# mabdullahsoyturk/Torch-Sputnik

Measured on AMD Instinct MI355X. Metric: SpMM effective GFLOP/s (2*nnz*N/t), M=N=K=4096 fp32, density 0.1, higher is better.
Workload: dtype f32

## Files before the change

torch_sputnik_amd/csrc/gen_spmm_flat.py:

```python
#!/usr/bin/env python3
import argparse

_ap = argparse.ArgumentParser()
_ap.add_argument("--mode", default="entry", choices=["entry", "group"])
_ap.add_argument("--layout", default="straight", choices=["straight", "diagonal"])
_ap.add_argument("out", nargs="?")
ARGS = _ap.parse_args()
GROUP = ARGS.mode == "group"

BK = 32
BK_SHIFT = 5
ROW_BYTES = 2048
ROW_SHIFT = 11
WIN_BYTES = 144
NSTRIP = 4
NPIECES = 4
ROWSTEP = 8

V_LANE, V_STAGE, V_PLAN, V_ROWS = "v0", "v1", "v2", "v3"
CUR_OFF, CUR_VAL = 4, 5
NXT_OFF, NXT_VAL, NXT_ROWS = 6, 7, 8
NN_OFF, NN_VAL, NN_ROWS = 10, 11, 12
PAIR = [16, 18, 20, 22]
VALT = [16, 18]
V_ADDR = 20
STRIP = [32, 40, 48, 56]
ACC = 64

S_STREAM, S_VALUES, S_CINFO, S_DENSE = "s[36:37]", "s[38:39]", "s[40:41]", "s[42:43]"
S_PITCH, S_KMAX, S_NCHUNKS, S_ROW0, S_LDS0, S_DEBUG = "s44", "s45", "s46", "s47", "s48", "s49"
S_REM, S_C, S_CIOFF, S_MINE, S_SB, S_NSW = "s50", "s51", "s56", "s57", "s76", "s77"
S_CI = ["s52", "s53", "s54", "s55"]
S_RET, S_BND = "s[58:59]", "s[60:61]"
S_ROWS = [62, 63, 64, 65]
S_IDX = [66, 67, 68, 69]
S_COLS = "s78"
S_T = ["s70", "s71", "s72", "s73", "s74", "s75"]

out = []


def emit(line):
    out.append(line)


def label(name):
    return f".L_{name}_%="


def strip_reads(ring, addr):
    s = STRIP[ring]
    emit(f"ds_read_b128 v[{s}:{s + 3}], v{addr}")
    emit(f"ds_read_b128 v[{s + 4}:{s + 7}], v{addr} offset:1024")


def fmas(src_pair, op_sel, ring):
    s = STRIP[ring]
    for q in range(4):
        emit(f"v_pk_fma_f32 v[{ACC + 2 * q}:{ACC + 2 * q + 1}], v[{src_pair}:{src_pair + 1}], "
             f"v[{s + 2 * q}:{s + 2 * q + 1}], v[{ACC + 2 * q}:{ACC + 2 * q + 1}] {op_sel}")


def entry_fma_stage(ring, lgkm):
    emit(f"s_waitcnt lgkmcnt({lgkm})")
    emit(f"s_set_gpr_idx_on s{S_IDX[ring]}, 0xc")
    fmas(PAIR[ring], "op_sel:[1,0,0] op_sel_hi:[1,1,1]", ring)
    emit("s_set_gpr_idx_off")


def entry_slot(slot):
    ring = slot % NSTRIP
    p = PAIR[ring]
    emit(f"{label(f'E_{slot}')}:")
    emit(f"s_sub_u32 {S_REM}, {S_REM}, 1")
    emit(f"s_cbranch_scc1 {label(f'bnd_{slot}')}")
    emit(f"v_mov_b64_dpp v[{p}:{p + 1}], v[{CUR_OFF}:{CUR_VAL}] row_newbcast:{slot} row_mask:0xf bank_mask:0xf")
    emit(f"s_bfe_u32 s{S_IDX[ring]}, s{S_ROWS[slot // 4]}, {hex(8 * (slot % 4) | (7 << 16))}")
    emit(f"v_add_u32 v{p}, v{p}, {V_LANE}")
    strip_reads(ring, p)
    entry_fma_stage((ring + 1) % NSTRIP, 2 * (NSTRIP - 1))


def group_entry_body(ring, slot):
    t = VALT[slot % 2]
    emit(f"v_mov_b32_dpp v{t}, v{CUR_VAL} row_newbcast:{slot} row_mask:0xf bank_mask:0xf")
    emit(f"s_bfe_u32 s{S_IDX[0]}, s{S_ROWS[slot // 4]}, {hex(8 * (slot % 4) | (7 << 16))}")
    emit(f"s_set_gpr_idx_on s{S_IDX[0]}, 0xc")
    fmas(t, "op_sel:[0,0,0] op_sel_hi:[0,1,1]", ring)
    emit("s_set_gpr_idx_off")


def group_start(ring, slot):
    emit(f"{label(f'N_{ring}_{slot}')}:")
    emit(f"s_sub_u32 {S_REM}, {S_REM}, 1")
    emit(f"s_cbranch_scc1 {label(f'bnd_{slot}')}")
    emit(f"v_mov_b32_dpp v{V_ADDR}, v{CUR_OFF} row_newbcast:{slot} row_mask:0xf bank_mask:0xf")
    emit(f"v_add_u32 v{V_ADDR}, v{V_ADDR}, {V_LANE}")
    strip_reads(ring, V_ADDR)
    emit(f"s_waitcnt lgkmcnt({2 * (NSTRIP - 1)})")


def first_groups():
    for i in range(NSTRIP - 1):
        emit(f"s_bfe_u32 {S_T[0]}, {S_COLS}, {hex(8 * i | (8 << 16))}")
        emit(f"s_lshl_b32 {S_T[0]}, {S_T[0]}, {ROW_SHIFT}")
        emit(f"v_add_u32 v{V_ADDR}, {S_T[0]}, {V_LANE}")
        strip_reads(i, V_ADDR)


def stage_chunk(chunk_sgpr):
    t_row, t_lds, t_r, t_lo, t_hi = S_T[1], S_T[2], S_T[3], S_T[4], S_T[5]
    emit(f"s_lshl_b32 {t_row}, {chunk_sgpr}, {BK_SHIFT}")
    emit(f"s_add_u32 {t_row}, {t_row}, {S_ROW0}")
    emit(f"s_and_b32 {t_lds}, {chunk_sgpr}, 1")
    emit(f"s_lshl_b32 {t_lds}, {t_lds}, 16")
    emit(f"s_add_u32 {t_lds}, {t_lds}, {S_LDS0}")
    for i in range(NPIECES):
        emit(f"s_add_u32 {t_r}, {t_row}, {ROWSTEP * i}")
        emit(f"s_min_u32 {t_r}, {t_r}, {S_KMAX}")
        emit(f"s_mul_hi_u32 {t_hi}, {t_r}, {S_PITCH}")
        emit(f"s_mul_i32 {t_lo}, {t_r}, {S_PITCH}")
        emit(f"s_add_u32 {t_lo}, {t_lo}, s42")
        emit(f"s_addc_u32 {t_hi}, {t_hi}, s43")
        emit(f"s_add_u32 m0, {t_lds}, {hex(ROWSTEP * i * ROW_BYTES)}")
        emit("s_nop 0")
        emit(f"global_load_lds_dwordx4 {V_STAGE}, s[{t_lo[1:]}:{t_hi[1:]}]")


def plan_load(off, rows):
    emit(f"global_load_dwordx2 v[{off}:{off + 1}], {V_PLAN}, {S_STREAM}")
    emit(f"global_load_dword v{rows}, {V_ROWS}, {S_STREAM}")
    emit(f"v_add_u32 {V_PLAN}, {hex(WIN_BYTES)}, {V_PLAN}")
    emit(f"v_add_u32 {V_ROWS}, {hex(WIN_BYTES)}, {V_ROWS}")


def gather(val):
    emit(f"global_load_dword v{val}, v{val}, {S_VALUES}")


def switch_window(tag):
    emit(f"s_cmp_lg_u32 {S_SB}, 0")
    emit(f"s_cbranch_scc1 {label('swc_' + tag)}")
    emit("s_waitcnt vmcnt(0)")
    emit(f"s_branch {label('swd_' + tag)}")
    emit(f"{label('swc_' + tag)}:")
    emit(f"s_waitcnt vmcnt({NPIECES})")
    emit(f"{label('swd_' + tag)}:")
    emit(f"s_mov_b32 {S_SB}, 0")
    emit(f"s_add_u32 {S_NSW}, {S_NSW}, 1")
    for i in range(4):
        emit(f"v_readlane_b32 s{S_ROWS[i]}, v{NXT_ROWS}, {i}")
    emit(f"v_bfe_u32 v{CUR_OFF}, v{NXT_OFF}, {8 if GROUP else 0}, 8")
    emit(f"v_mov_b32 v{CUR_VAL}, v{NXT_VAL}")
    emit(f"v_lshlrev_b32 v{CUR_OFF}, {ROW_SHIFT}, v{CUR_OFF}")
    emit(f"v_mov_b64 v[{NXT_OFF}:{NXT_VAL}], v[{NN_OFF}:{NN_VAL}]")
    emit(f"v_mov_b32 v{NXT_ROWS}, v{NN_ROWS}")
    emit(f"s_bitcmp1_b32 {S_DEBUG}, 3")
    emit(f"s_cbranch_scc1 {label('swskip_' + tag)}")
    gather(NXT_VAL)
    plan_load(NN_OFF, NN_ROWS)
    emit(f"{label('swskip_' + tag)}:")
    emit("s_nop 1")


def take_chunk_info():
    emit(f"s_mov_b32 {S_REM}, {S_CI[0] if GROUP else S_CI[3]}")
    if GROUP:
        emit(f"s_mov_b32 {S_COLS}, {S_CI[1]}")


def generate():
    emit("; ---- prologue ----")
    for r in list(range(ACC, ACC + 64)) + list(range(STRIP[0], STRIP[0] + 32)) + list(range(16, 24)):
        emit(f"v_mov_b32 v{r}, 0")
    for r in S_IDX:
        emit(f"s_mov_b32 s{r}, 0")
    emit(f"s_getpc_b64 {S_BND}")
    emit(f"{label('pc')}:")
    emit(f"s_add_u32 s60, s60, {label('boundary')}-{label('pc')}")
    emit("s_addc_u32 s61, s61, 0")
    plan_load(NXT_OFF, NXT_ROWS)
    plan_load(NN_OFF, NN_ROWS)
    emit("s_waitcnt vmcnt(2)")
    gather(NXT_VAL)
    emit(f"s_mov_b32 {S_T[0]}, 0")
    stage_chunk(S_T[0])
    emit(f"s_load_dwordx4 s[52:55], {S_CINFO}, 0x0")
    emit("s_waitcnt vmcnt(0) lgkmcnt(0)")
    emit("s_barrier")
    take_chunk_info()
    emit(f"s_load_dwordx4 s[52:55], {S_CINFO}, 0x10")
    emit(f"s_mov_b32 {S_CIOFF}, 32")
    emit(f"s_mov_b32 {S_C}, 0")
    emit(f"s_mov_b32 {S_NSW}, 0")
    emit(f"s_mov_b32 {S_SB}, 0")
    emit(f"s_mov_b32 {S_MINE}, 0")
    if GROUP:
        first_groups()
    emit(f"s_cmp_lt_u32 {S_NCHUNKS}, 2")
    emit(f"s_cbranch_scc1 {label('pro_nostage')}")
    emit(f"s_mov_b32 {S_T[0]}, 1")
    stage_chunk(S_T[0])
    emit(f"s_mov_b32 {S_SB}, 1")
    emit(f"s_mov_b32 {S_MINE}, 1")
    emit(f"{label('pro_nostage')}:")
    switch_window("pro")

    emit("; ---- main loop ----")
    if not GROUP:
        for slot in range(16):
            entry_slot(slot)
        switch_window("w")
        emit(f"s_branch {label('E_0')}")
    elif ARGS.layout == "straight":
        emit(f"s_branch {label(f'E_{NSTRIP - 1}_0')}")
        for ring in range(NSTRIP):
            for slot in range(16):
                emit(f"{label(f'E_{ring}_{slot}')}:")
                emit(f"s_bitcmp1_b32 s{S_ROWS[slot // 4]}, {8 * (slot % 4) + 7}")
                emit(f"s_cbranch_scc1 {label(f'N_{ring}_{slot}')}")
                emit(f"{label(f'B_{ring}_{slot}')}:")
                group_entry_body(ring, slot)
            switch_window(f"r{ring}")
            emit(f"s_branch {label(f'E_{ring}_0')}")
        emit("; ---- first entry of a column group ----")
        for ring in range(NSTRIP):
            for slot in range(16):
                group_start(ring, slot)
                emit(f"s_branch {label(f'B_{(ring + 1) % NSTRIP}_{slot}')}")
    else:
        emit(f"s_branch {label(f'E_{NSTRIP - 1}_0')}")
        for diag in range(NSTRIP):
            for slot in range(16):
                ring = (diag + slot) % NSTRIP
                emit(f"{label(f'E_{ring}_{slot}')}:")
                emit(f"s_bitcmp1_b32 s{S_ROWS[slot // 4]}, {8 * (slot % 4) + 7}")
                emit(f"s_cbranch_scc0 {label(f'B_{ring}_{slot}')}")
                group_start(ring, slot)
                emit(f"{label(f'B_{(ring + 1) % NSTRIP}_{slot}')}:")
                group_entry_body((ring + 1) % NSTRIP, slot)
            ring = (diag + 16) % NSTRIP
            switch_window(f"r{diag}")
            emit(f"s_branch {label(f'E_{ring}_0')}")

    emit("; ---- boundary stubs ----")
    for slot in range(16):
        emit(f"{label(f'bnd_{slot}')}:")
        emit(f"s_swappc_b64 {S_RET}, {S_BND}")
        if GROUP:
            emit(f"s_cbranch_scc1 {label('end')}")
            emit(f"s_branch {label(f'N_{NSTRIP - 1}_{slot}')}")
        else:
            emit(f"s_cbranch_scc1 {label(f'drain_{slot % NSTRIP}')}")
            emit(f"s_branch {label(f'E_{slot}')}")

    emit("; ---- boundary subroutine ----")
    emit(f"{label('boundary')}:")
    emit(f"s_bitcmp1_b32 {S_DEBUG}, 2")
    emit(f"s_cbranch_scc1 {label('bnodrain')}")
    emit("s_waitcnt lgkmcnt(0)")
    emit(f"{label('bnodrain')}:")
    emit(f"s_cmp_eq_u32 {S_MINE}, 0")
    emit(f"s_cbranch_scc1 {label('bvd')}")
    emit(f"s_bitcmp1_b32 {S_DEBUG}, 5")
    emit(f"s_cbranch_scc1 {label('bvd')}")
    for n in range(3):
        emit(f"s_cmp_eq_u32 {S_NSW}, {n}")
        emit(f"s_cbranch_scc1 {label(f'bv{n}')}")
    emit("s_waitcnt vmcnt(9)")
    emit(f"s_branch {label('bvd')}")
    for n in range(3):
        emit(f"{label(f'bv{n}')}:")
        emit(f"s_waitcnt vmcnt({3 * n})")
        if n < 2:
            emit(f"s_branch {label('bvd')}")
    emit(f"{label('bvd')}:")
    emit(f"s_bitcmp1_b32 {S_DEBUG}, 1")
    emit(f"s_cbranch_scc1 {label('bnobar')}")
    emit("s_barrier")
    emit(f"{label('bnobar')}:")
    emit(f"s_add_u32 {S_C}, {S_C}, 1")
    emit(f"s_cmp_eq_u32 {S_C}, {S_NCHUNKS}")
    emit(f"s_cbranch_scc1 {label('bret')}")
    take_chunk_info()
    emit(f"s_load_dwordx4 s[52:55], {S_CINFO}, {S_CIOFF}")
    emit(f"s_add_u32 {S_CIOFF}, {S_CIOFF}, 16")
    if GROUP:
        first_groups()
    emit(f"s_mov_b32 {S_NSW}, 0")
    emit(f"s_mov_b32 {S_MINE}, 0")
    emit(f"s_add_u32 {S_T[0]}, {S_C}, 1")
    emit(f"s_cmp_ge_u32 {S_T[0]}, {S_NCHUNKS}")
    emit(f"s_cbranch_scc1 {label('bnostage')}")
    emit(f"s_bitcmp1_b32 {S_DEBUG}, 0")
    emit(f"s_cbranch_scc1 {label('bnostage')}")
    stage_chunk(S_T[0])
    emit(f"s_add_u32 {S_SB}, {S_SB}, 1")
    emit(f"s_mov_b32 {S_MINE}, 1")
    emit(f"{label('bnostage')}:")
    emit(f"s_cmp_eq_u32 {S_C}, {S_NCHUNKS}")
    emit(f"{label('bret')}:")
    emit(f"s_setpc_b64 {S_RET}")

    if not GROUP:
        emit("; ---- drain: the three entries still in the pipeline ----")
        for ring in range(NSTRIP):
            emit(f"{label(f'drain_{ring}')}:")
            for j in range(1, NSTRIP):
                entry_fma_stage((ring + j) % NSTRIP, 2 * (NSTRIP - 1 - j))
            if ring < NSTRIP - 1:
                emit(f"s_branch {label('end')}")
    emit(f"{label('end')}:")
    emit("s_waitcnt vmcnt(0) lgkmcnt(0)")


def main():
    generate()
    text = "// GENERATED by gen_spmm_flat.py -- do not edit.\n" + "".join(
        f'"{line}\\n"\n' for line in out)
    if ARGS.out:
        with open(ARGS.out, "w") as f:
            f.write(text)
    else:
        print(text, end="")


if __name__ == "__main__":
    main()
```

torch_sputnik_amd/csrc/spmm_flat.hip:

```cpp
#include <algorithm>

#include "options.h"
#include "spmm_tiled_common.h"

namespace sputnik_hip {

namespace {

using namespace tiled;

constexpr int kBN = 512;
constexpr int kBK = 32;
constexpr int kWaves = 16;
constexpr int kRPW = 8;
constexpr int kBM = kWaves * kRPW;
constexpr int kAhead = 3;
constexpr int kDealPer = 256;
constexpr int kWindow = 16;
constexpr int kWindowBytes = 144;
constexpr int kTailWindows = 4;
constexpr int kMaxColumns = 65536;
constexpr unsigned kNewGroup = 0x80;


struct ChunkInfo {
  int groups;
  unsigned first_rows;
  unsigned unused;
  int entries;
};

__host__ __device__ inline size_t fill_tables_bytes(int nchunks) {
  return (sizeof(int) * (static_cast<size_t>(nchunks) * (kBK / 4 + 4) + 2 * kRPW + 2) + 15) / 16 * 16;
}
__device__ __forceinline__ int wave_sum(int v) {
#pragma unroll
  for (int o = 32; o > 0; o >>= 1) v += __shfl_xor(v, o);
  return v;
}
__device__ __forceinline__ int wave_inclusive_scan(int v, int lane) {
#pragma unroll
  for (int o = 1; o < 64; o <<= 1) {
    const int t = __shfl_up(v, o);
    if (lane >= o) v += t;
  }
  return v;
}

__global__ __launch_bounds__(kRPW * 64) void spmm_flat_fill_kernel(
    int m, int k, int slots, int nchunks, const int* __restrict__ row_indices,
    const int* __restrict__ row_offsets, const int* __restrict__ column_indices,
    int* __restrict__ row_ok, ChunkInfo* __restrict__ cinfo, int* __restrict__ gwin,
    unsigned char* __restrict__ stream, int stage_windows, int debug) {
  extern __shared__ unsigned lds[];
  constexpr int RPW = kRPW, BK = kBK, NT = RPW * 64;
  constexpr int WPC = BK / 4;
  constexpr int UN = 4;
  const int g = blockIdx.x, tid = threadIdx.x, lane = tid % 64, wave = tid / 64;
  const int groups = gridDim.x;
  unsigned* maskw = lds;
  int* ebase = reinterpret_cast<int*>(lds + nchunks * WPC);
  unsigned* nzmask = reinterpret_cast<unsigned*>(ebase + nchunks);
  unsigned* wprefix = nzmask + nchunks;
  int* scratch = reinterpret_cast<int*>(wprefix + 2 * nchunks);
  unsigned char* sbuf = reinterpret_cast<unsigned char*>(lds) + fill_tables_bytes(nchunks);

  for (int i = tid; i < nchunks * WPC; i += NT) maskw[i] = 0;
  const int slot = g * RPW + wave;
  const int entry = dealt_index(slot, slots, kDealPer);
  int p0 = 0, p1 = 0;
  if (entry < m) {
    const int row = row_indices[entry];
    p0 = row_offsets[row];
    p1 = row_offsets[row + 1];
  }
  int before = 0;
  for (int gp = tid; gp < g; gp += NT) {
    int rows[RPW], len = 0;
    int2 bounds[RPW];
#pragma unroll
    for (int r = 0; r < RPW; ++r) {
      const int e = dealt_index(gp * RPW + r, slots, kDealPer);
      rows[r] = e < m ? row_indices[e] : -1;
    }
#pragma unroll
    for (int r = 0; r < RPW; ++r) {
      typedef int int2_a4 __attribute__((ext_vector_type(2), aligned(4)));
      if (rows[r] >= 0) {
        const int2_a4 pair = *reinterpret_cast<const int2_a4*>(row_offsets + rows[r]);
        bounds[r] = make_int2(pair.x, pair.y);
      } else {
        bounds[r] = make_int2(0, 0);
      }
    }
#pragma unroll
    for (int r = 0; r < RPW; ++r) len += bounds[r].y - bounds[r].x;
    before += (len + kWindow - 1) / kWindow;
  }
  before = wave_sum(before);
  if (lane == 0) {
    scratch[wave] = before;
    scratch[RPW + wave] = p1 - p0;
  }
  if (tid == 0) scratch[2 * RPW] = 1;
  __syncthreads();
  int wbase = 0, total = 0;
#pragma unroll
  for (int r = 0; r < RPW; ++r) {
    wbase += scratch[r];
    total += scratch[RPW + r];
  }
  if (tid == 0) gwin[g] = wbase;
  unsigned char* my_stream = stream + static_cast<int64_t>(wbase) * kWindowBytes;
  const int windows = (total + kWindow - 1) / kWindow;

  bool ok = true;
  for (int base = p0; base < p1; base += 64 * UN) {
    int cur[UN], prev[UN];
#pragma unroll
    for (int u = 0; u < UN; ++u) {
      const int p = base + u * 64 + lane;
      cur[u] = p < p1 ? column_indices[p] : -2;
    }
    const int before_base = base > p0 ? column_indices[base - 1] : -1;
#pragma unroll
    for (int u = 0; u < UN; ++u) {
      const int up = __shfl_up(cur[u], 1);
      const int carry = u == 0 ? before_base : __shfl(cur[u == 0 ? 0 : u - 1], 63);
      prev[u] = lane == 0 ? carry : up;
    }
#pragma unroll
    for (int u = 0; u < UN; ++u) {
      if (cur[u] == -2) continue;
      if (cur[u] <= prev[u] || cur[u] >= k) ok = false;
      else atomicOr(&maskw[cur[u] >> 2], (1u << wave) << (8 * (cur[u] & 3)));
    }
  }
  const bool wave_ok = __builtin_amdgcn_ballot_w64(!ok) == 0;
  if (lane == 0) {
    row_ok[slot] = wave_ok ? 1 : 0;
    if (!wave_ok) scratch[2 * RPW] = 0;
  }
  __syncthreads();
  ChunkInfo* my_info = cinfo + static_cast<int64_t>(g) * (nchunks + 1);
  if (scratch[2 * RPW] == 0) {
    unsigned* w = reinterpret_cast<unsigned*>(my_stream);
    const int nwin = windows + (g == groups - 1 ? kTailWindows : 0);
    for (int i = tid; i < nwin * (kWindowBytes / 4); i += NT)
      w[i] = i % (kWindowBytes / 4) >= 32 ? 0x80808080u : 0u;
    for (int c = tid; c <= nchunks; c += NT) my_info[c] = ChunkInfo{0, 0u, 0u, 0};
    return;
  }

  if (debug & 0x100) return;
  for (int t0 = 0; t0 < nchunks * WPC; t0 += NT) {
    const int t = t0 + tid;
    const bool live = t < nchunks * WPC;
    const int c = t / WPC, i = t % WPC;
    const unsigned w = live ? maskw[t] : 0u;
    const int cnt = __popc(w);
    unsigned nz = 0u;
#pragma unroll
    for (int b = 0; b < 4; ++b)
      if ((w >> (8 * b)) & 0xffu) nz |= 1u << (4 * i + b);
    int incl = cnt;
#pragma unroll
    for (int o = 1; o < WPC; o <<= 1) {
      const int up = __shfl_up(incl, o, WPC);
      if (i >= o) incl += up;
    }
#pragma unroll
    for (int o = 1; o < WPC; o <<= 1) nz |= static_cast<unsigned>(__shfl_xor(static_cast<int>(nz), o, WPC));
    const int entries = __shfl(incl, WPC - 1, WPC);
    if (live) {
      reinterpret_cast<unsigned char*>(wprefix)[t] = static_cast<unsigned char>(incl - cnt);
      if (i == 0) {
        unsigned first = 0u, rest = nz;
        const int cgroups = __popc(nz);
#pragma unroll
        for (int q = 0; q < kAhead; ++q)
          if (rest) {
            first |= static_cast<unsigned>((c & 1) * BK + __ffs(rest) - 1) << (8 * q);
            rest &= rest - 1u;
          }
        ebase[c] = entries;
        nzmask[c] = nz;
        my_info[c] = ChunkInfo{cgroups, first, 0u, entries};
      }
    }
  }
  if (tid == 0) my_info[nchunks] = ChunkInfo{0, 0u, 0u, 0};
  __syncthreads();
  if (wave == 0) {
    int carry = 0;
    for (int c0 = 0; c0 < nchunks; c0 += 64) {
      const int c = c0 + lane;
      const int e = c < nchunks ? ebase[c] : 0;
      const int incl = wave_inclusive_scan(e, lane);
      if (c < nchunks) ebase[c] = carry + incl - e;
      carry += __shfl(incl, 63);
    }
  }
  __syncthreads();

  if (debug & 0x200) return;
  static_assert(WPC == 8, "two prefix words per chunk");
  const int nwin_out = windows + (g == groups - 1 ? kTailWindows : 0);
  const bool staged = nwin_out <= stage_windows && !(debug & 0x1000);
  unsigned char* const dst_stream = staged ? sbuf : my_stream;
  for (int base = p0; base < p1; base += 64 * UN) {
    int cols[UN];
#pragma unroll
    for (int u = 0; u < UN; ++u) {
      const int p = base + u * 64 + lane;
      cols[u] = p < p1 ? column_indices[p] : -1;
    }
#pragma unroll
    for (int u = 0; u < UN; ++u) {
      if (cols[u] < 0) continue;
      const int p = base + u * 64 + lane;
      const int col = cols[u], c = col / BK, j = col % BK;
      const unsigned w = maskw[c * WPC + j / 4];
      const int prefix = static_cast<int>((wprefix[2 * c + j / 16] >> (8 * ((j / 4) % 4))) & 0xffu) +
                         __popc(w & ((1u << (8 * (j & 3))) - 1u));
      const unsigned byte = (w >> (8 * (j & 3))) & 0xffu;
      const int own = __popc(byte & ((1u << wave) - 1u));
      const int pos = ebase[c] + prefix + own;
      unsigned rowbyte = wave * 8, tile_rows = static_cast<unsigned>((c & 1) * BK + j);
      if (own == 0) {
        rowbyte |= kNewGroup;
        unsigned ahead = j == BK - 1 ? 0u : nzmask[c] >> (j + 1);
        ahead &= ahead - 1u;
        ahead &= ahead - 1u;
        if (ahead) tile_rows |= static_cast<unsigned>((c & 1) * BK + j + __ffs(ahead)) << 8;
      }
      if (debug & 0x400) continue;
      unsigned char* block = dst_stream + static_cast<int64_t>(pos / kWindow) * kWindowBytes;
      const int e = pos % kWindow;
      *reinterpret_cast<uint2*>(block + 8 * e) = make_uint2(tile_rows, static_cast<unsigned>(p) * 4u);
      block[128 + e] = static_cast<unsigned char>(rowbyte);
    }
  }
  for (int pos = total + tid; pos < windows * kWindow; pos += NT) {
    unsigned char* block = dst_stream + static_cast<int64_t>(pos / kWindow) * kWindowBytes;
    *reinterpret_cast<uint2*>(block + 8 * (pos % kWindow)) = make_uint2(0u, 0u);
    block[128 + pos % kWindow] = static_cast<unsigned char>(kNewGroup);
  }
  if (g == groups - 1) {
    unsigned* w = reinterpret_cast<unsigned*>(dst_stream + static_cast<int64_t>(windows) * kWindowBytes);
    for (int i = tid; i < kTailWindows * (kWindowBytes / 4); i += NT)
      w[i] = i % (kWindowBytes / 4) >= 32 ? 0x80808080u : 0u;
  }
  if (staged) {
    __syncthreads();
    const uint4* src = reinterpret_cast<const uint4*>(sbuf);
    uint4* dst = reinterpret_cast<uint4*>(my_stream);
    for (int i = tid; i < nwin_out * (kWindowBytes / 16); i += NT) dst[i] = src[i];
  }
}

using v8f = float __attribute__((ext_vector_type(8)));

#define SPUTNIK_HIP_FLAT_ASM_OPERANDS                                                              \
      : "={v[64:71]}"(a0), "={v[72:79]}"(a1), "={v[80:87]}"(a2), "={v[88:95]}"(a3),                \
        "={v[96:103]}"(a4), "={v[104:111]}"(a5), "={v[112:119]}"(a6), "={v[120:127]}"(a7)          \
      : "{v0}"(lane_base), "{v1}"(stage_off), "{v2}"(plan_off), "{v3}"(rows_off),                  \
        "{s[36:37]}"(my_stream), "{s[38:39]}"(values), "{s[40:41]}"(my_info), "{s[42:43]}"(dense), \
        "{s44}"(pitch), "{s45}"(kmax), "{s46}"(nchunks), "{s47}"(row0), "{s48}"(lds0),             \
        "{s49}"(debug)                                                                             \
      : "memory", "m0", "scc", "v4", "v5", "v6", "v7", "v8", "v9", "v10", "v11", "v12", "v13",     \
        "v14", "v15", "v16", "v17", "v18", "v19", "v20", "v21", "v22", "v23", "v32", "v33", "v34", \
        "v35", "v36", "v37", "v38", "v39", "v40", "v41", "v42", "v43", "v44", "v45", "v46", "v47", \
        "v48", "v49", "v50", "v51", "v52", "v53", "v54", "v55", "v56", "v57", "v58", "v59", "v60", \
        "v61", "v62", "v63", "s50", "s51", "s52", "s53", "s54", "s55", "s56", "s57", "s58", "s59", \
        "s60", "s61", "s62", "s63", "s64", "s65", "s66", "s67", "s68", "s69", "s70", "s71", "s72", \
        "s73", "s74", "s75", "s76", "s77", "s78", "s79", "s80"

template <int LOOP>
__global__ __launch_bounds__(kWaves * 64) void spmm_flat_kernel(
    int m, int k, int n, int slots, int nchunks, int n_tiles, const int* __restrict__ row_indices,
    const float* __restrict__ values, int64_t values_stride, const ChunkInfo* __restrict__ cinfo,
    const int* __restrict__ gwin, const unsigned char* __restrict__ stream,
    const float* __restrict__ dense, int64_t dense_stride, float* __restrict__ out,
    int64_t out_stride, const int* __restrict__ row_ok, const int* __restrict__ row_offsets,
    const int* __restrict__ column_indices, int debug, Epilogue epi) {
  constexpr int RPW = kRPW, BM = kBM, BN = kBN, BK = kBK, VEC = 8;
  constexpr int PPR = VEC / 4;
  __shared__ float tile[2][BK * BN];

  const int lane = threadIdx.x % kWave;
  const int wave = __builtin_amdgcn_readfirstlane(threadIdx.x / kWave);

  const int bid = blockIdx.x;
  int ntile, mblock;
  int replica = blockIdx.y;
  const int xcd_cols = 1 << ((debug >> 13) & 3);
  if (xcd_cols > 1 && n_tiles == 8 && (gridDim.x / 8) % xcd_cols == 0) {
    const int xcd = bid % 8, i = bid / 8, col_groups = 8 / xcd_cols;
    ntile = (xcd % col_groups) * xcd_cols + i % xcd_cols;
    mblock = (xcd / col_groups) * ((gridDim.x / 8) / xcd_cols) + i / xcd_cols;
  } else if (n_tiles % 8 == 0) {
    const int per_xcd = n_tiles / 8;
    const int xcd = bid % 8, i = bid / 8;
    ntile = xcd * per_xcd + i % per_xcd;
    mblock = i / per_xcd;
  } else {
    const int work = xcd_local_index32();
    const int mblocks = gridDim.x / n_tiles;
    mblock = work % mblocks;
    ntile = (work / mblocks) % n_tiles;
    replica = work / (mblocks * n_tiles);
  }
  values += replica * values_stride;
  dense += replica * dense_stride;
  out += replica * out_stride;

  const int n0 = ntile * BN;
  const int slot0 = mblock * BM + wave * RPW;

  if (!block_rows_ok_wave(row_ok, mblock * BM, BM)) {
    for (int r = 0; r < RPW; ++r) {
      const int entry = dealt_index(slot0 + r, slots, kDealPer);
      if (entry >= m) continue;
      const int row = row_indices[entry];
#pragma unroll
      for (int h = 0; h < PPR; ++h) {
        if (n0 + h * 256 + lane * 4 >= n) continue;
        const int col = min(n0 + h * 256 + lane * 4, n - 4);
        const float4 acc4 = gather_row_strip(values, column_indices, row_offsets[row],
                                             row_offsets[row + 1], dense + col, n);
        *reinterpret_cast<float4*>(out + static_cast<int64_t>(row) * n + col) =
            apply_epilogue(acc4, epi, row);
      }
    }
    return;
  }

  const int group = slot0 / RPW;
  const unsigned char* my_stream =
      stream + static_cast<int64_t>(__builtin_amdgcn_readfirstlane(gwin[group])) * kWindowBytes;
  const ChunkInfo* my_info = cinfo + static_cast<int64_t>(group) * (nchunks + 1);
  const unsigned tile_lds = static_cast<unsigned>(reinterpret_cast<uintptr_t>(AS_LDS(&tile[0][0])));
  const unsigned lane_base = tile_lds + lane * 16;
  const unsigned stage_off =
      static_cast<unsigned>(min(n0 + (wave % PPR) * 256 + lane * 4, n - 4)) * 4u;
  const unsigned plan_off = (lane & 15) * 8, rows_off = 128 + (lane & 3) * 4;
  const int pitch = n * 4, kmax = k - 1, row0 = wave / PPR;
  const int lds0 = static_cast<int>(tile_lds) + (wave / PPR) * (BN * 4) + (wave % PPR) * 1024;

  v8f a0, a1, a2, a3, a4, a5, a6, a7;
  if constexpr (LOOP == 0) {
    asm volatile(
#include "spmm_flat_body_entry.inc"
        SPUTNIK_HIP_FLAT_ASM_OPERANDS);
  } else if constexpr (LOOP == 1) {
    asm volatile(
#include "spmm_flat_body_group_s.inc"
        SPUTNIK_HIP_FLAT_ASM_OPERANDS);
  } else {
    asm volatile(
#include "spmm_flat_body_group_d.inc"
        SPUTNIK_HIP_FLAT_ASM_OPERANDS);
  }

  const v8f acc[8] = {a0, a1, a2, a3, a4, a5, a6, a7};
#pragma unroll
  for (int r = 0; r < RPW; ++r) {
    const int entry = dealt_index(slot0 + r, slots, kDealPer);
    if (entry < m) {
      const int row = row_indices[entry];
#pragma unroll
      for (int h = 0; h < PPR; ++h)
        if (n0 + h * 256 + lane * 4 < n) {
          const int col = min(n0 + h * 256 + lane * 4, n - 4);
          const int f = r * VEC + 4 * h;
          *reinterpret_cast<float4*>(out + static_cast<int64_t>(row) * n + col) =
              apply_epilogue(make_float4(acc[f / 8][f % 8], acc[f / 8][f % 8 + 1],
                                         acc[f / 8][f % 8 + 2], acc[f / 8][f % 8 + 3]),
                             epi, row);
        }
    }
  }
}

struct FlatPlan {
  int slots, nchunks, n_tiles, groups;
  size_t row_ok_off, cinfo_off, gwin_off, stream_off, bytes;
};

FlatPlan make_flat_plan(int m, int k, int n, int nonzeros) {
  FlatPlan p;
  p.slots = ceil_div(m, kDealPer) * kDealPer;
  p.nchunks = ceil_div(k, kBK);
  p.n_tiles = ceil_div(n, kBN);
  p.groups = p.slots / kRPW;
  auto up = [](size_t v) { return (v + 255) / 256 * 256; };
  p.row_ok_off = 0;
  p.cinfo_off = row_ok_bytes(p.slots);
  p.gwin_off = up(p.cinfo_off + sizeof(ChunkInfo) * static_cast<size_t>(p.nchunks + 1) * p.groups);
  p.stream_off = up(p.gwin_off + sizeof(int) * static_cast<size_t>(p.groups));
  const size_t windows = static_cast<size_t>(nonzeros) / kWindow + p.groups + kTailWindows;
  p.bytes = up(p.stream_off + windows * kWindowBytes);
  return p;
}

int fill_stage_windows(int nchunks, int nonzeros, int groups) {
  const size_t tables = fill_tables_bytes(nchunks);
  if (tables + kWindowBytes > 64 * 1024) return 0;
  const int64_t room = static_cast<int64_t>((64 * 1024 - tables) / kWindowBytes);
  const int64_t want = (static_cast<int64_t>(nonzeros) / kWindow / groups) * 5 / 4 + kTailWindows + 2;
  return static_cast<int>(std::min(room, want));
}
size_t fill_lds_bytes(int nchunks, int stage_windows) {
  return fill_tables_bytes(nchunks) + static_cast<size_t>(stage_windows) * kWindowBytes;
}

int flat_mode(int m, int k, int nonzeros) {
  const int forced = options().spmm_sparse;
  if (forced >= 2 && forced <= 4) return forced - 2;
  const double d = static_cast<double>(nonzeros) / (static_cast<double>(m) * k);
  return d < 0.12 ? 0 : d < 0.36 ? 2 : 1;
}

}

static bool fill_lds_available(int k) {
  static const bool extended = [] {
    return hipFuncSetAttribute(reinterpret_cast<const void*>(spmm_flat_fill_kernel),
                               hipFuncAttributeMaxDynamicSharedMemorySize,
                               static_cast<int>(fill_lds_bytes(kMaxColumns / kBK, 0))) == hipSuccess;
  }();
  return extended || fill_lds_bytes(ceil_div(k, kBK), 0) <= 64 * 1024;
}

bool spmm_flat_applicable(int m, int k, int n, int nonzeros) {
  if (n < 4 || k < kBK || m < 64 || nonzeros < 16 * static_cast<int64_t>(m) ||
      nonzeros >= (1 << 29))
    return false;
  if (static_cast<int64_t>(ceil_div(n, kBN)) * kBN * 3 > static_cast<int64_t>(n) * 4) return false;
  return k <= kMaxColumns && m <= 16384 && fill_lds_available(k);
}

const char* spmm_flat_kernel_name(int m, int k, int nonzeros) {
  static const char* const names[] = {"spmm_flat_kernel<0>", "spmm_flat_kernel<1>", "spmm_flat_kernel<2>"};
  return names[flat_mode(m, k, nonzeros)];
}

int64_t spmm_flat_tiles(int m, int n) {
  return static_cast<int64_t>(ceil_div(m, kBM)) * ceil_div(n, kBN);
}

size_t spmm_flat_workspace_bytes(int m, int k, int n, int nonzeros) {
  return make_flat_plan(m, k, n, nonzeros).bytes;
}

int spmm_flat_plan(int m, int k, int n, int nonzeros, const int* row_indices,
                   const int* row_offsets, const int* column_indices, void* workspace,
                   hipStream_t stream) {
  const FlatPlan p = make_flat_plan(m, k, n, nonzeros);
  char* base = static_cast<char*>(workspace);
  if (!fill_lds_available(k)) return SPUTNIK_HIP_UNSUPPORTED;
  const int stage_windows = fill_stage_windows(p.nchunks, nonzeros, p.groups);
  hipLaunchKernelGGL(spmm_flat_fill_kernel, dim3(p.groups), dim3(kRPW * 64),
                     fill_lds_bytes(p.nchunks, stage_windows), stream, m, k, p.slots, p.nchunks, row_indices,
                     row_offsets, column_indices, reinterpret_cast<int*>(base + p.row_ok_off),
                     reinterpret_cast<ChunkInfo*>(base + p.cinfo_off),
                     reinterpret_cast<int*>(base + p.gwin_off),
                     reinterpret_cast<unsigned char*>(base + p.stream_off), stage_windows,
                     options().spmm_debug);
  return launch_status();
}

int xcd_columns_code(int k, int n, int nonzeros, int row_blocks) {
  const int forced = options().spmm_debug;
  if (forced & 0x8000) return (forced >> 13) & 3;
  if (ceil_div(n, kBN) != 8) return 0;
  const double stream = 13.0 * nonzeros, b = 4.0 * k * n;
  int best = 0;
  double best_bytes = stream * 8 + b;
  for (int code = 1; code <= 3; ++code) {
    const int c = 1 << code;
    if (row_blocks % c != 0) break;
    const double bytes = stream * 8 / c + b * c;
    if (bytes < 0.97 * best_bytes) {
      best = code;
      best_bytes = bytes;
    }
  }
  return best;
}

int spmm_flat_exec(int m, int k, int n, int nonzeros, int replicas, const int* row_indices,
                   const float* values, int64_t values_stride, const int* row_offsets,
                   const int* column_indices, const float* dense, int64_t dense_stride, float* out,
                   int64_t out_stride, const void* workspace, hipStream_t stream, Epilogue epi) {
  const FlatPlan p = make_flat_plan(m, k, n, nonzeros);
  const char* base = static_cast<const char*>(workspace);
#define SPUTNIK_HIP_LAUNCH_FLAT(LOOP)                                                              \
  hipLaunchKernelGGL((spmm_flat_kernel<LOOP>), dim3((p.slots / kBM) * p.n_tiles, replicas),        \
                     dim3(kWaves * 64), 0, stream, m, k, n, p.slots, p.nchunks, p.n_tiles,         \
                     row_indices, values, values_stride,                                           \
                     reinterpret_cast<const ChunkInfo*>(base + p.cinfo_off),                       \
                     reinterpret_cast<const int*>(base + p.gwin_off),                              \
                     reinterpret_cast<const unsigned char*>(base + p.stream_off), dense,           \
                     dense_stride, out, out_stride,                                                \
                     reinterpret_cast<const int*>(base + p.row_ok_off), row_offsets,               \
                     column_indices, debug_word, epi)
  const int debug_word = (options().spmm_debug & ~0xe000) |
                         (xcd_columns_code(k, n, nonzeros, p.slots / kBM) << 13);
  switch (flat_mode(m, k, nonzeros)) {
    case 0: SPUTNIK_HIP_LAUNCH_FLAT(0); break;
    case 1: SPUTNIK_HIP_LAUNCH_FLAT(1); break;
    default: SPUTNIK_HIP_LAUNCH_FLAT(2); break;
  }
#undef SPUTNIK_HIP_LAUNCH_FLAT
  return launch_status();
}

}
```

Measured before the change: 42960.

## Add scalar-metadata SpMM loop variant with compact 64-byte stream windows

```diff
diff --git a/torch_sputnik_amd/csrc/gen_spmm_flat.py b/torch_sputnik_amd/csrc/gen_spmm_flat.py
--- a/torch_sputnik_amd/csrc/gen_spmm_flat.py
+++ b/torch_sputnik_amd/csrc/gen_spmm_flat.py
@@ -2,11 +2,12 @@
 import argparse
 
 _ap = argparse.ArgumentParser()
-_ap.add_argument("--mode", default="entry", choices=["entry", "group"])
+_ap.add_argument("--mode", default="entry", choices=["entry", "group", "scalar"])
 _ap.add_argument("--layout", default="straight", choices=["straight", "diagonal"])
 _ap.add_argument("out", nargs="?")
 ARGS = _ap.parse_args()
 GROUP = ARGS.mode == "group"
+SCALAR = ARGS.mode == "scalar"
 
 BK = 32
 BK_SHIFT = 5
@@ -36,6 +37,23 @@
 S_IDX = [66, 67, 68, 69]
 S_COLS = "s78"
 S_T = ["s70", "s71", "s72", "s73", "s74", "s75"]
+
+
+SC_WIN = 8
+SC_WIN_BYTES = 64
+SC_PAR = 2
+SC_META = [52, 60]
+V_LANEM = "v21"
+V_VOA = "v22"
+V_VOFF, V_VALN, V_VALC = 23, 24, 25
+VALT = [16, 18]
+if SCALAR:
+    S_SB, S_NSW = "s72", "s73"
+    S_CI = ["s84", "s85"]
+    S_RET, S_BND = "s[86:87]", "s[88:89]"
+    S_CIOFF, S_MINE, S_WOFF, S_G = "s90", "s91", "s92", "s94"
+    S_T = ["s96", "s97", "s98", "s99", "s100", "s101"]
+    S_COLS = S_T[5]
 
 out = []
 
@@ -164,8 +182,8 @@
 
 
 def take_chunk_info():
-    emit(f"s_mov_b32 {S_REM}, {S_CI[0] if GROUP else S_CI[3]}")
-    if GROUP:
+    emit(f"s_mov_b32 {S_REM}, {S_CI[0] if GROUP or SCALAR else S_CI[3]}")
+    if GROUP or SCALAR:
         emit(f"s_mov_b32 {S_COLS}, {S_CI[1]}")
 
 
@@ -314,8 +332,168 @@
     emit("s_waitcnt vmcnt(0) lgkmcnt(0)")
 
 
+
+
+def sc_slot(par, ring, slot):
+    w = f"s{SC_META[par] + slot}"
+    emit(f"{label(f'E_{par}_{ring}_{slot}')}:")
+    emit(f"s_bfe_u32 {S_G}, {w}, {hex(8 | (8 << 16))}")
+    emit(f"s_cbranch_scc0 {label(f'B_{par}_{ring}_{slot}')}")
+    emit(f"{label(f'N_{par}_{ring}_{slot}')}:")
+    emit(f"s_sub_u32 {S_REM}, {S_REM}, 1")
+    emit(f"s_cbranch_scc1 {label(f'bnd_{par}_{slot}')}")
+    emit(f"v_lshl_add_u32 v{V_ADDR}, {S_G}, {ROW_SHIFT}, {V_LANEM}")
+    strip_reads(ring, V_ADDR)
+    if slot >= NSTRIP - 1:
+        emit(f"s_waitcnt lgkmcnt({2 * (NSTRIP - 1)})")
+    nxt = (ring + 1) % NSTRIP
+    emit(f"{label(f'B_{par}_{nxt}_{slot}')}:")
+    t = VALT[slot % 2]
+    emit(f"v_mov_b32_dpp v{t}, v{V_VALC} row_newbcast:{slot} row_mask:0xf bank_mask:0xf")
+    emit(f"s_set_gpr_idx_on {w}, 0xc")
+    fmas_s(f"v[{t}:{t + 1}]", "op_sel:[0,0,0] op_sel_hi:[0,1,1]", nxt)
+    emit("s_set_gpr_idx_off")
+
+
+def fmas_s(src, op_sel, ring):
+    s = STRIP[ring]
+    for q in range(4):
+        emit(f"v_pk_fma_f32 v[{ACC + 2 * q}:{ACC + 2 * q + 1}], {src}, "
+             f"v[{s + 2 * q}:{s + 2 * q + 1}], v[{ACC + 2 * q}:{ACC + 2 * q + 1}] {op_sel}")
+
+
+def sc_switch(par, tag):
+    emit(f"s_cmp_lg_u32 {S_SB}, 0")
+    emit(f"s_cbranch_scc1 {label('swc_' + tag)}")
+    emit("s_waitcnt vmcnt(0) lgkmcnt(0)")
+    emit(f"s_branch {label('swd_' + tag)}")
+    emit(f"{label('swc_' + tag)}:")
+    emit(f"s_waitcnt vmcnt({NPIECES}) lgkmcnt(0)")
+    emit(f"{label('swd_' + tag)}:")
+    emit(f"s_mov_b32 {S_SB}, 0")
+    emit(f"s_add_u32 {S_NSW}, {S_NSW}, 1")
+    emit(f"v_mov_b32 v{V_VALC}, v{V_VALN}")
+    emit(f"global_load_dword v{V_VALN}, v{V_VOFF}, {S_VALUES}")
+    emit(f"v_add_u32 {V_VOA}, {hex(SC_WIN_BYTES)}, {V_VOA}")
+    emit(f"global_load_dword v{V_VOFF}, {V_VOA}, {S_STREAM}")
+    emit(f"s_load_dwordx8 s[{SC_META[par]}:{SC_META[par] + 7}], {S_STREAM}, {S_WOFF}")
+    emit(f"s_add_u32 {S_WOFF}, {S_WOFF}, {hex(SC_WIN_BYTES)}")
+    emit("s_nop 1")
+
+
+def generate_scalar():
+    emit("; ---- prologue ----")
+    for r in list(range(ACC, ACC + 64)) + list(range(STRIP[0], STRIP[0] + 32)):
+        emit(f"v_mov_b32 v{r}, 0")
+    emit(f"v_add_u32 {V_LANEM}, {hex(-(1 << ROW_SHIFT) & 0xffffffff)}, {V_LANE}")
+    emit(f"s_getpc_b64 {S_BND}")
+    emit(f"{label('pc')}:")
+    lo, hi = S_BND[2:-1].split(":")
+    emit(f"s_add_u32 s{lo}, s{lo}, {label('boundary')}-{label('pc')}")
+    emit(f"s_addc_u32 s{hi}, s{hi}, 0")
+    emit(f"v_lshrrev_b32 {V_VOA}, 1, {V_PLAN}")
+    emit(f"v_and_b32 {V_VOA}, 28, {V_VOA}")
+    emit(f"v_add_u32 {V_VOA}, 32, {V_VOA}")
+    emit(f"s_mov_b32 {S_T[0]}, 0")
+    stage_chunk(S_T[0])
+    emit(f"s_load_dwordx2 s[{S_CI[0][1:]}:{S_CI[1][1:]}], {S_CINFO}, 0x0")
+    for w, dst in ((0, V_VALC), (1, V_VALN)):
+        emit(f"global_load_dword v{V_VOFF}, {V_VOA}, {S_STREAM}")
+        emit("s_waitcnt vmcnt(0)")
+        emit(f"global_load_dword v{dst}, v{V_VOFF}, {S_VALUES}")
+        emit(f"v_add_u32 {V_VOA}, {hex(SC_WIN_BYTES)}, {V_VOA}")
+    emit("s_waitcnt vmcnt(0)")
+    emit(f"global_load_dword v{V_VOFF}, {V_VOA}, {S_STREAM}")
+    for w in range(SC_PAR):
+        emit(f"s_load_dwordx8 s[{SC_META[w]}:{SC_META[w] + 7}], {S_STREAM}, {hex(w * SC_WIN_BYTES)}")
+    emit(f"s_mov_b32 {S_WOFF}, {hex(SC_PAR * SC_WIN_BYTES)}")
+    emit("s_waitcnt vmcnt(0) lgkmcnt(0)")
+    emit("s_barrier")
+    take_chunk_info()
+    emit(f"s_load_dwordx2 s[{S_CI[0][1:]}:{S_CI[1][1:]}], {S_CINFO}, 0x10")
+    emit(f"s_mov_b32 {S_CIOFF}, 32")
+    emit(f"s_mov_b32 {S_C}, 0")
+    emit(f"s_mov_b32 {S_MINE}, 0")
+    emit(f"s_mov_b32 {S_SB}, 0")
+    emit(f"s_mov_b32 {S_NSW}, 0")
+    first_groups()
+    emit(f"s_cmp_lt_u32 {S_NCHUNKS}, 2")
+    emit(f"s_cbranch_scc1 {label('pro_nostage')}")
+    emit(f"s_mov_b32 {S_T[0]}, 1")
+    stage_chunk(S_T[0])
+    emit(f"s_mov_b32 {S_MINE}, 1")
+    emit(f"s_mov_b32 {S_SB}, 1")
+    emit(f"{label('pro_nostage')}:")
+    emit("s_waitcnt lgkmcnt(0)")
+    emit(f"s_branch {label(f'E_0_{NSTRIP - 1}_0')}")
+
+    emit("; ---- main loop: two window parities x four diagonals ----")
+    for par in range(SC_PAR):
+        for diag in range(NSTRIP):
+            for slot in range(SC_WIN):
+                sc_slot(par, (diag + slot) % NSTRIP, slot)
+            sc_switch(par, f"{par}_{diag}")
+            emit(f"s_branch {label(f'E_{(par + 1) % SC_PAR}_{(diag + SC_WIN) % NSTRIP}_0')}")
+
+    emit("; ---- boundary stubs ----")
+    for par in range(SC_PAR):
+        for slot in range(SC_WIN):
+            emit(f"{label(f'bnd_{par}_{slot}')}:")
+            emit(f"s_swappc_b64 {S_RET}, {S_BND}")
+            if slot < NSTRIP - 1:
+                emit(f"s_waitcnt lgkmcnt({2 * slot})")
+            emit(f"s_cbranch_scc1 {label('end')}")
+            emit(f"s_branch {label(f'N_{par}_{NSTRIP - 1}_{slot}')}")
+
+    emit("; ---- boundary subroutine ----")
+    emit(f"{label('boundary')}:")
+    emit("s_waitcnt lgkmcnt(0)")
+    emit(f"s_cmp_eq_u32 {S_MINE}, 0")
+    emit(f"s_cbranch_scc1 {label('bvd')}")
+    emit(f"s_bitcmp1_b32 {S_DEBUG}, 5")
+    emit(f"s_cbranch_scc1 {label('bvd')}")
+    for n in range(2):
+        emit(f"s_cmp_eq_u32 {S_NSW}, {n}")
+        emit(f"s_cbranch_scc1 {label(f'bv{n}')}")
+    emit("s_waitcnt vmcnt(4)")
+    emit(f"s_branch {label('bvd')}")
+    for n in range(2):
+        emit(f"{label(f'bv{n}')}:")
+        emit(f"s_waitcnt vmcnt({2 * n})")
+        if n < 1:
+            emit(f"s_branch {label('bvd')}")
+    emit(f"{label('bvd')}:")
+    emit(f"s_bitcmp1_b32 {S_DEBUG}, 1")
+    emit(f"s_cbranch_scc1 {label('bnobar')}")
+    emit("s_barrier")
+    emit(f"{label('bnobar')}:")
+    emit(f"s_add_u32 {S_C}, {S_C}, 1")
+    emit(f"s_cmp_eq_u32 {S_C}, {S_NCHUNKS}")
+    emit(f"s_cbranch_scc1 {label('bret')}")
+    take_chunk_info()
+    emit(f"s_load_dwordx2 s[{S_CI[0][1:]}:{S_CI[1][1:]}], {S_CINFO}, {S_CIOFF}")
+    emit(f"s_add_u32 {S_CIOFF}, {S_CIOFF}, 16")
+    first_groups()
+    emit(f"s_mov_b32 {S_MINE}, 0")
+    emit(f"s_mov_b32 {S_NSW}, 0")
+    emit(f"s_add_u32 {S_T[0]}, {S_C}, 1")
+    emit(f"s_cmp_ge_u32 {S_T[0]}, {S_NCHUNKS}")
+    emit(f"s_cbranch_scc1 {label('bnostage')}")
+    emit(f"s_bitcmp1_b32 {S_DEBUG}, 0")
+    emit(f"s_cbranch_scc1 {label('bnostage')}")
+    stage_chunk(S_T[0])
+    emit(f"s_add_u32 {S_SB}, {S_SB}, 1")
+    emit(f"s_mov_b32 {S_MINE}, 1")
+    emit(f"{label('bnostage')}:")
+    emit(f"s_cmp_eq_u32 {S_C}, {S_NCHUNKS}")
+    emit(f"{label('bret')}:")
+    emit(f"s_setpc_b64 {S_RET}")
+    emit(f"{label('end')}:")
+    emit("s_waitcnt vmcnt(0) lgkmcnt(0)")
+
+
 def main():
-    generate()
+    generate_scalar() if SCALAR else generate()
     text = "// GENERATED by gen_spmm_flat.py -- do not edit.\n" + "".join(
         f'"{line}\\n"\n' for line in out)
     if ARGS.out:
diff --git a/torch_sputnik_amd/csrc/spmm_flat.hip b/torch_sputnik_amd/csrc/spmm_flat.hip
--- a/torch_sputnik_amd/csrc/spmm_flat.hip
+++ b/torch_sputnik_amd/csrc/spmm_flat.hip
@@ -21,6 +21,9 @@
 constexpr int kTailWindows = 4;
 constexpr int kMaxColumns = 65536;
 constexpr unsigned kNewGroup = 0x80;
+constexpr int kScWindow = 8;
+constexpr int kScWindowBytes = 64;
+constexpr unsigned kScPad = 0x0100u;
 
 
 struct ChunkInfo {
@@ -47,6 +50,7 @@
   return v;
 }
 
+template <bool SC>
 __global__ __launch_bounds__(kRPW * 64) void spmm_flat_fill_kernel(
     int m, int k, int slots, int nchunks, const int* __restrict__ row_indices,
     const int* __restrict__ row_offsets, const int* __restrict__ column_indices,
@@ -54,6 +58,12 @@
     unsigned char* __restrict__ stream, int stage_windows, int debug) {
   extern __shared__ unsigned lds[];
   constexpr int RPW = kRPW, BK = kBK, NT = RPW * 64;
+  constexpr int kWindow = SC ? kScWindow : ::sputnik_hip::kWindow;
+  constexpr int kWindowBytes = SC ? kScWindowBytes : ::sputnik_hip::kWindowBytes;
+  auto pad_word = [](int i) -> unsigned {
+    return SC ? (i % (kWindowBytes / 4) < kScWindow ? kScPad : 0u)
+              : (i % (kWindowBytes / 4) >= 32 ? 0x80808080u : 0u);
+  };
   constexpr int WPC = BK / 4;
   constexpr int UN = 4;
   const int g = blockIdx.x, tid = threadIdx.x, lane = tid % 64, wave = tid / 64;
@@ -146,8 +156,7 @@
   if (scratch[2 * RPW] == 0) {
     unsigned* w = reinterpret_cast<unsigned*>(my_stream);
     const int nwin = windows + (g == groups - 1 ? kTailWindows : 0);
-    for (int i = tid; i < nwin * (kWindowBytes / 4); i += NT)
-      w[i] = i % (kWindowBytes / 4) >= 32 ? 0x80808080u : 0u;
+    for (int i = tid; i < nwin * (kWindowBytes / 4); i += NT) w[i] = pad_word(i);
     for (int c = tid; c <= nchunks; c += NT) my_info[c] = ChunkInfo{0, 0u, 0u, 0};
     return;
   }
@@ -237,19 +246,29 @@
       if (debug & 0x400) continue;
       unsigned char* block = dst_stream + static_cast<int64_t>(pos / kWindow) * kWindowBytes;
       const int e = pos % kWindow;
-      *reinterpret_cast<uint2*>(block + 8 * e) = make_uint2(tile_rows, static_cast<unsigned>(p) * 4u);
-      block[128 + e] = static_cast<unsigned char>(rowbyte);
+      if constexpr (SC) {
+        const unsigned field = own == 0 ? 1u + (tile_rows >> 8) : 0u;
+        *reinterpret_cast<unsigned*>(block + 4 * e) = static_cast<unsigned>(wave * 8) | field << 8;
+        *reinterpret_cast<unsigned*>(block + 32 + 4 * e) = static_cast<unsigned>(p) * 4u;
+      } else {
+        *reinterpret_cast<uint2*>(block + 8 * e) = make_uint2(tile_rows, static_cast<unsigned>(p) * 4u);
+        block[128 + e] = static_cast<unsigned char>(rowbyte);
+      }
     }
   }
   for (int pos = total + tid; pos < windows * kWindow; pos += NT) {
     unsigned char* block = dst_stream + static_cast<int64_t>(pos / kWindow) * kWindowBytes;
-    *reinterpret_cast<uint2*>(block + 8 * (pos % kWindow)) = make_uint2(0u, 0u);
-    block[128 + pos % kWindow] = static_cast<unsigned char>(kNewGroup);
+    if constexpr (SC) {
+      *reinterpret_cast<unsigned*>(block + 4 * (pos % kWindow)) = kScPad;
+      *reinterpret_cast<unsigned*>(block + 32 + 4 * (pos % kWindow)) = 0u;
+    } else {
+      *reinterpret_cast<uint2*>(block + 8 * (pos % kWindow)) = make_uint2(0u, 0u);
+      block[128 + pos % kWindow] = static_cast<unsigned char>(kNewGroup);
+    }
   }
   if (g == groups - 1) {
     unsigned* w = reinterpret_cast<unsigned*>(dst_stream + static_cast<int64_t>(windows) * kWindowBytes);
-    for (int i = tid; i < kTailWindows * (kWindowBytes / 4); i += NT)
-      w[i] = i % (kWindowBytes / 4) >= 32 ? 0x80808080u : 0u;
+    for (int i = tid; i < kTailWindows * (kWindowBytes / 4); i += NT) w[i] = pad_word(i);
   }
   if (staged) {
     __syncthreads();
@@ -275,6 +294,24 @@
         "v61", "v62", "v63", "s50", "s51", "s52", "s53", "s54", "s55", "s56", "s57", "s58", "s59", \
         "s60", "s61", "s62", "s63", "s64", "s65", "s66", "s67", "s68", "s69", "s70", "s71", "s72", \
         "s73", "s74", "s75", "s76", "s77", "s78", "s79", "s80"
+
+#define SPUTNIK_HIP_FLAT_SCALAR_ASM_OPERANDS                                                       \
+      : "={v[64:71]}"(a0), "={v[72:79]}"(a1), "={v[80:87]}"(a2), "={v[88:95]}"(a3),                \
+        "={v[96:103]}"(a4), "={v[104:111]}"(a5), "={v[112:119]}"(a6), "={v[120:127]}"(a7)          \
+      : "{v0}"(lane_base), "{v1}"(stage_off), "{v2}"(plan_off), "{v3}"(rows_off),                  \
+        "{s[36:37]}"(my_stream), "{s[38:39]}"(values), "{s[40:41]}"(my_info), "{s[42:43]}"(dense), \
+        "{s44}"(pitch), "{s45}"(kmax), "{s46}"(nchunks), "{s47}"(row0), "{s48}"(lds0),             \
+        "{s49}"(debug)                                                                             \
+      : "memory", "m0", "scc", "v4", "v5", "v6", "v7", "v8", "v9", "v10", "v11", "v12", "v13",    \
+        "v14", "v15", "v16", "v17", "v18", "v19", "v20", "v21", "v22", "v23", "v24", "v25", "v26", \
+        "v27", "v28", "v29", "v32", "v33", "v34", "v35", "v36",                                    \
+        "v37", "v38", "v39", "v40", "v41", "v42", "v43", "v44", "v45", "v46", "v47", "v48", "v49", \
+        "v50", "v51", "v52", "v53", "v54", "v55", "v56", "v57", "v58", "v59", "v60", "v61", "v62", \
+        "v63", "s50", "s51",                                                                       \
+        "s52", "s53", "s54", "s55", "s56", "s57", "s58", "s59", "s60", "s61", "s62", "s63", "s64", \
+        "s65", "s66", "s67", "s68", "s69", "s70", "s71", "s72", "s73", "s74", "s75", "s76", "s77", \
+        "s78", "s79", "s80", "s81", "s82", "s83", "s84", "s85", "s86", "s87", "s88", "s89", "s90", \
+        "s91", "s92", "s93", "s94", "s95", "s96", "s97", "s98", "s99", "s100", "s101"
 
 template <int LOOP>
 __global__ __launch_bounds__(kWaves * 64) void spmm_flat_kernel(
@@ -338,7 +375,8 @@
 
   const int group = slot0 / RPW;
   const unsigned char* my_stream =
-      stream + static_cast<int64_t>(__builtin_amdgcn_readfirstlane(gwin[group])) * kWindowBytes;
+      stream + static_cast<int64_t>(__builtin_amdgcn_readfirstlane(gwin[group])) *
+                   (LOOP == 3 ? kScWindowBytes : kWindowBytes);
   const ChunkInfo* my_info = cinfo + static_cast<int64_t>(group) * (nchunks + 1);
   const unsigned tile_lds = static_cast<unsigned>(reinterpret_cast<uintptr_t>(AS_LDS(&tile[0][0])));
   const unsigned lane_base = tile_lds + lane * 16;
@@ -357,10 +395,14 @@
     asm volatile(
 #include "spmm_flat_body_group_s.inc"
         SPUTNIK_HIP_FLAT_ASM_OPERANDS);
-  } else {
+  } else if constexpr (LOOP == 2) {
     asm volatile(
 #include "spmm_flat_body_group_d.inc"
         SPUTNIK_HIP_FLAT_ASM_OPERANDS);
+  } else {
+    asm volatile(
+#include "spmm_flat_body_scalar.inc"
+        SPUTNIK_HIP_FLAT_SCALAR_ASM_OPERANDS);
   }
 
   const v8f acc[8] = {a0, a1, a2, a3, a4, a5, a6, a7};
@@ -383,13 +425,25 @@
   }
 }
 
+int flat_mode(int m, int k, int nonzeros) {
+  const int forced = options().spmm_sparse;
+  if (forced >= 2 && forced <= 5) return forced - 2;
+  const double d = static_cast<double>(nonzeros) / (static_cast<double>(m) * k);
+  return d < 0.07 ? 0 : 3;
+}
+
 struct FlatPlan {
   int slots, nchunks, n_tiles, groups;
+  bool scalar;
+  int window, window_bytes;
   size_t row_ok_off, cinfo_off, gwin_off, stream_off, bytes;
 };
 
 FlatPlan make_flat_plan(int m, int k, int n, int nonzeros) {
   FlatPlan p;
+  p.scalar = flat_mode(m, k, nonzeros) == 3;
+  p.window = p.scalar ? kScWindow : kWindow;
+  p.window_bytes = p.scalar ? kScWindowBytes : kWindowBytes;
   p.slots = ceil_div(m, kDealPer) * kDealPer;
   p.nchunks = ceil_div(k, kBK);
   p.n_tiles = ceil_div(n, kBN);
@@ -399,36 +453,31 @@
   p.cinfo_off = row_ok_bytes(p.slots);
   p.gwin_off = up(p.cinfo_off + sizeof(ChunkInfo) * static_cast<size_t>(p.nchunks + 1) * p.groups);
   p.stream_off = up(p.gwin_off + sizeof(int) * static_cast<size_t>(p.groups));
-  const size_t windows = static_cast<size_t>(nonzeros) / kWindow + p.groups + kTailWindows;
-  p.bytes = up(p.stream_off + windows * kWindowBytes);
+  const size_t windows = static_cast<size_t>(nonzeros) / p.window + p.groups + kTailWindows;
+  p.bytes = up(p.stream_off + windows * p.window_bytes);
   return p;
 }
 
-int fill_stage_windows(int nchunks, int nonzeros, int groups) {
+int fill_stage_windows(int nchunks, int nonzeros, int groups, int window, int window_bytes) {
   const size_t tables = fill_tables_bytes(nchunks);
-  if (tables + kWindowBytes > 64 * 1024) return 0;
-  const int64_t room = static_cast<int64_t>((64 * 1024 - tables) / kWindowBytes);
-  const int64_t want = (static_cast<int64_t>(nonzeros) / kWindow / groups) * 5 / 4 + kTailWindows + 2;
+  if (tables + window_bytes > 64 * 1024) return 0;
+  const int64_t room = static_cast<int64_t>((64 * 1024 - tables) / window_bytes);
+  const int64_t want = (static_cast<int64_t>(nonzeros) / window / groups) * 5 / 4 + kTailWindows + 2;
   return static_cast<int>(std::min(room, want));
 }
-size_t fill_lds_bytes(int nchunks, int stage_windows) {
-  return fill_tables_bytes(nchunks) + static_cast<size_t>(stage_windows) * kWindowBytes;
-}
-
-int flat_mode(int m, int k, int nonzeros) {
-  const int forced = options().spmm_sparse;
-  if (forced >= 2 && forced <= 4) return forced - 2;
-  const double d = static_cast<double>(nonzeros) / (static_cast<double>(m) * k);
-  return d < 0.12 ? 0 : d < 0.36 ? 2 : 1;
+size_t fill_lds_bytes(int nchunks, int stage_windows, int window_bytes = kWindowBytes) {
+  return fill_tables_bytes(nchunks) + static_cast<size_t>(stage_windows) * window_bytes;
 }
 
 }
 
 static bool fill_lds_available(int k) {
   static const bool extended = [] {
-    return hipFuncSetAttribute(reinterpret_cast<const void*>(spmm_flat_fill_kernel),
-                               hipFuncAttributeMaxDynamicSharedMemorySize,
-                               static_cast<int>(fill_lds_bytes(kMaxColumns / kBK, 0))) == hipSuccess;
+    const int bytes = static_cast<int>(fill_lds_bytes(kMaxColumns / kBK, 0));
+    return hipFuncSetAttribute(reinterpret_cast<const void*>(spmm_flat_fill_kernel<false>),
+                               hipFuncAttributeMaxDynamicSharedMemorySize, bytes) == hipSuccess &&
+           hipFuncSetAttribute(reinterpret_cast<const void*>(spmm_flat_fill_kernel<true>),
+                               hipFuncAttributeMaxDynamicSharedMemorySize, bytes) == hipSuccess;
   }();
   return extended || fill_lds_bytes(ceil_div(k, kBK), 0) <= 64 * 1024;
 }
@@ -442,7 +491,8 @@
 }
 
 const char* spmm_flat_kernel_name(int m, int k, int nonzeros) {
-  static const char* const names[] = {"spmm_flat_kernel<0>", "spmm_flat_kernel<1>", "spmm_flat_kernel<2>"};
+  static const char* const names[] = {"spmm_flat_kernel<0>", "spmm_flat_kernel<1>", "spmm_flat_kernel<2>",
+                                      "spmm_flat_kernel<3>"};
   return names[flat_mode(m, k, nonzeros)];
 }
 
@@ -460,10 +510,12 @@
   const FlatPlan p = make_flat_plan(m, k, n, nonzeros);
   char* base = static_cast<char*>(workspace);
   if (!fill_lds_available(k)) return SPUTNIK_HIP_UNSUPPORTED;
-  const int stage_windows = fill_stage_windows(p.nchunks, nonzeros, p.groups);
-  hipLaunchKernelGGL(spmm_flat_fill_kernel, dim3(p.groups), dim3(kRPW * 64),
-                     fill_lds_bytes(p.nchunks, stage_windows), stream, m, k, p.slots, p.nchunks, row_indices,
-                     row_offsets, column_indices, reinterpret_cast<int*>(base + p.row_ok_off),
+  const int stage_windows = fill_stage_windows(p.nchunks, nonzeros, p.groups, p.window, p.window_bytes);
+  hipLaunchKernelGGL(p.scalar ? spmm_flat_fill_kernel<true> : spmm_flat_fill_kernel<false>,
+                     dim3(p.groups), dim3(kRPW * 64),
+                     fill_lds_bytes(p.nchunks, stage_windows, p.window_bytes), stream, m, k, p.slots,
+                     p.nchunks, row_indices, row_offsets, column_indices,
+                     reinterpret_cast<int*>(base + p.row_ok_off),
                      reinterpret_cast<ChunkInfo*>(base + p.cinfo_off),
                      reinterpret_cast<int*>(base + p.gwin_off),
                      reinterpret_cast<unsigned char*>(base + p.stream_off), stage_windows,
@@ -511,7 +563,8 @@
   switch (flat_mode(m, k, nonzeros)) {
     case 0: SPUTNIK_HIP_LAUNCH_FLAT(0); break;
     case 1: SPUTNIK_HIP_LAUNCH_FLAT(1); break;
-    default: SPUTNIK_HIP_LAUNCH_FLAT(2); break;
+    case 2: SPUTNIK_HIP_LAUNCH_FLAT(2); break;
+    default: SPUTNIK_HIP_LAUNCH_FLAT(3); break;
   }
 #undef SPUTNIK_HIP_LAUNCH_FLAT
   return launch_status();
```

Result: no change. 43150 (median of 6 runs) (+0.4%).
